# weiwei-ww/ML-VAE

Hardware: AMD Instinct MI355X
Metric: spectrogram frames/sec + ELBO; 80-d log-mel B=256 at 1/2/4/8 MI355X (higher is better)
Workload: dtype bf16

## Files before the change

ml-vae_amd/csrc/heads.hip:

```cpp
#include "common.h"
#include <stdlib.h>

namespace {

constexpr float LOG_2PI_H = 1.8378770351409912f;
constexpr int RT = 64;

struct HeadArgs {
  int B, T, N, H2, loss_type, train;
  const unsigned short* Y;
  const unsigned short* W1;
  const unsigned short* W1t;
  const float* b1;
  const float* W2[2]; const float* b2[2]; const float* W3[2]; const float* b3[2];
  const float* x; const float* lens; const int* count; float rec_scale;
  float* P1; float* P2[2]; float* OUT[2]; float* dOUT[2]; float* dP2[2]; float* dP1; float* dY;
  float* partials;
  int sbf;
  float* bias_ws;
  float* wg_ws;
};

template <int C, int F> constexpr int nbs() { return 2 * F + 2 * C + 2 * C; }

// ... 360 lines not shown
      for (int idx = tid; idx < 2 * (FK - F) * LC; idx += 256)
        sm[O_W3I + (idx / ((FK - F) * LC)) * W3R * LC + F * LC + idx % ((FK - F) * LC)] = 0;
    } else {
      for (int idx = tid; idx < 2 * C * (FK - F); idx += 256) {
        const int h = idx / (C * (FK - F)), rem = idx % (C * (FK - F));
        sm[O_W3T + h * C * LF + (rem / (FK - F)) * LF + F + rem % (FK - F)] = 0;
      }
    }
    for (int idx = tid; idx < 2 * RT * (FK - F); idx += 256) {
      const int h = idx / (RT * (FK - F)), rem = idx % (RT * (FK - F));
      sm[O_DO + h * RT * LF + (rem / (FK - F)) * LF + F + rem % (FK - F)] = 0;
    }
  }
  {
    __shared__ int cnt_sh;
    const int c = block_frames(a.lens, a.B, a.T, a.count, &cnt_sh);
    if (tid == 0) inv_cnt = c > 0 ? 1.f / ((float)c * (float)F) : 0.f;
  }

  const unsigned short* P1b = reinterpret_cast<const unsigned short*>(a.P1);
  u32x4 pn[4];
  f32x4 xn[NF];
  float lnn;
  auto prefetch = [&](int tile) {
    const int grow = tile * RT + 16 * wave + l15;
    const bool rv = tile < ntiles && grow < a.N;
    lnn = rv ? a.lens[grow / a.T] : 0.f;
#pragma unroll
    for (int i = 0; i < 4; ++i)
      pn[i] = rv ? *reinterpret_cast<const u32x4*>(P1b + (size_t)grow * C2 + 8 * (q + 4 * i)) : u32x4{0u, 0u, 0u, 0u};
#pragma unroll
    for (int j = 0; j < NF; ++j)
      xn[j] = rv ? *reinterpret_cast<const f32x4*>(a.x + (size_t)grow * F + 16 * j + 4 * q) : f32x4{0.f, 0.f, 0.f, 0.f};
  };
  prefetch(blockIdx.x);
  for (int i = tid; i < 2 * C; i += 256) sbias[i] = a.b2[i / C] ? a.b2[i / C][i % C] : 0.f;
  for (int i = tid; i < 2 * F; i += 256) sbias[2 * C + i] = a.b3[i / F] ? a.b3[i / F][i % F] : 0.f;
  __syncthreads();

  const int lrow = 16 * wave + l15;
  constexpr int NT3W = nt3<C, F>() / 4, NT2W = nt2<C, F>() / 4;
  static_assert(nt3<C, F>() % 4 == 0 && nt2<C, F>() % 4 == 0, "tiles split over 4 waves");
  f32x4 aw3[WG ? NT3W : 1], aw2[WG ? NT2W : 1];
  if constexpr (WG) {
#pragma unroll
    for (int i = 0; i < NT3W; ++i) aw3[i] = f32x4{0.f, 0.f, 0.f, 0.f};
#pragma unroll
    for (int i = 0; i < NT2W; ++i) aw2[i] = f32x4{0.f, 0.f, 0.f, 0.f};
  }
  constexpr bool SAVE = !WG;
  for (int tile = blockIdx.x; tile < ntiles; tile += gridDim.x) {
    const int grow = tile * RT + lrow;
    const bool rv = grow < a.N;
    const float lenb = lnn;
#pragma unroll
    for (int i = 0; i < 4; ++i) *reinterpret_cast<u32x4*>(sm + O_P1 + lrow * L2C + 8 * (q + 4 * i)) = pn[i];
    f32x4 xv[NF];
#pragma unroll
    for (int j = 0; j < NF; ++j) xv[j] = xn[j];
    prefetch(tile + gridDim.x);
    f32x4 p1r[NC2];
#pragma unroll
    for (int j = 0; j < NC2; ++j) {
      const bf16x4 v = *reinterpret_cast<const bf16x4*>(sm + O_P1 + lrow * L2C + 16 * j + 4 * q);
#pragma unroll
      for (int r = 0; r < 4; ++r) p1r[j][r] = bf2f(v[r]);
    }

    f32x4 acc2[2][NC], acc3[2][NF];
#pragma unroll
    for (int h = 0; h < 2; ++h) {
#pragma unroll
      for (int j = 0; j < NC; ++j) acc2[h][j] = f32x4{0.f, 0.f, 0.f, 0.f};
#pragma unroll
      for (int kk = 0; kk < C; kk += 32) {
        const bf16x8 av = lds8(sm + O_P1 + lrow * L2C + h * C + kk + 8 * q);
#pragma unroll
        for (int j = 0; j < NC; ++j) {
          acc2[h][j] = mfma16(lds8(sm + O_W2I + h * C * LC + (16 * j + l15) * LC + kk + 8 * q), av, acc2[h][j]);
          if constexpr (SPL)
            acc2[h][j] = mfma16(lds8(sm + O_W2T + h * C * LC + (16 * j + l15) * LC + kk + 8 * q), av, acc2[h][j]);
        }
      }
#pragma unroll
      for (int j = 0; j < NC; ++j) {
        const int col = 16 * j + 4 * q;
        const f32x4 bb = *reinterpret_cast<const f32x4*>(sbias + h * C + col);
#pragma unroll
        for (int r = 0; r < 4; ++r) acc2[h][j][r] = lrelu(acc2[h][j][r] + bb[r]);
        st4bf(sm + O_P2 + h * RT * LC + lrow * LC + col, acc2[h][j]);
        if (SAVE && rv) st_saved(a.P2[h], (size_t)grow * C + col, acc2[h][j], 1);
      }
#pragma unroll
      for (int j = 0; j < NF; ++j) acc3[h][j] = f32x4{0.f, 0.f, 0.f, 0.f};
#pragma unroll
      for (int kk = 0; kk < C; kk += 32) {
        const bf16x8 av = lds8(sm + O_P2 + h * RT * LC + lrow * LC + kk + 8 * q);
#pragma unroll
        for (int j = 0; j < NF; ++j) {
          const short* wr = sm + O_W3I + h * W3R * LC + (16 * j + l15) * LC;
          acc3[h][j] = mfma16(lds8(wr + kk + 8 * q), av, acc3[h][j]);
          if constexpr (SPL) {
            acc3[h][j] = mfma16(lds8(sm + O_W3T + h * F * LC + (16 * j + l15) * LC + kk + 8 * q), av, acc3[h][j]);
            const int s2 = kk / 32;
            const bf16x8 pl = {f2bf_lo(acc2[h][2 * s2][0]), f2bf_lo(acc2[h][2 * s2][1]),
                               f2bf_lo(acc2[h][2 * s2][2]), f2bf_lo(acc2[h][2 * s2][3]),
                               f2bf_lo(acc2[h][2 * s2 + 1][0]), f2bf_lo(acc2[h][2 * s2 + 1][1]),
                               f2bf_lo(acc2[h][2 * s2 + 1][2]), f2bf_lo(acc2[h][2 * s2 + 1][3])};
            const bf16x4 w0 = *reinterpret_cast<const bf16x4*>(wr + kk + 4 * q);
            const bf16x4 w1 = *reinterpret_cast<const bf16x4*>(wr + kk + 16 + 4 * q);
            acc3[h][j] = mfma16(bf16x8{w0[0], w0[1], w0[2], w0[3], w1[0], w1[1], w1[2], w1[3]}, pl, acc3[h][j]);
          }
        }
      }
#pragma unroll
      for (int j = 0; j < NF; ++j) {
        const int col = 16 * j + 4 * q;
        const f32x4 bb = *reinterpret_cast<const f32x4*>(sbias + 2 * C + h * F + col);
#pragma unroll
        for (int r = 0; r < 4; ++r) acc3[h][j][r] += bb[r];
        if (rv) *reinterpret_cast<f32x4*>(a.OUT[h] + (size_t)grow * F + col) = acc3[h][j];
      }
    }

    bool m = false;
    if (rv) m = grow % a.T < valid_frames(lenb, a.T);
    const float sc = m ? a.rec_scale * inv_cnt : 0.f;
    float lsum = 0.f;
#pragma unroll
    for (int j = 0; j < NF; ++j) {
      const int col = 16 * j + 4 * q;
      f32x4 gm, gv;
#pragma unroll
      for (int r = 0; r < 4; ++r) {
        const float mu = acc3[0][j][r], d = xv[j][r] - mu;
        float rr, gmu, glv = 0.f;
        if (lik) {
          const float lv = acc3[1][j][r];
          const float elv = expf(lv), ev = elv + 1e-5f;
          rr = 0.5f * (LOG_2PI_H + lv + d * d / ev);
          gmu = -d / ev;
          glv = 0.5f * (1.f - d * d * elv / (ev * ev));
        } else {
          rr = d * d;
          gmu = -2.f * d;
        }
        if (m) lsum += rr;
        gm[r] = sc * gmu;
        gv[r] = sc * glv;
      }
      rows16_to_lds(gm, &bred[wave][16 * j], lane);
      rows16_to_lds(gv, &bred[wave][F + 16 * j], lane);
      st4bf(sm + O_DO + lrow * LF + col, gm);
      st4bf(sm + O_DO + RT * LF + lrow * LF + col, gv);
      if (SAVE && rv) {
        st_saved(a.dOUT[0], (size_t)grow * F + col, gm, 1);
        if (lik) st_saved(a.dOUT[1], (size_t)grow * F + col, gv, 1);
      }
    }
    lsum = wave_sum(lsum);
    if (lane == 0) red[wave] = lsum;
    if constexpr (WG) {
      lds_barrier();
#pragma unroll
      for (int i = 0; i < NT3W; ++i) {
        const int t = wave * NT3W + i, h = t / ((F / 16) * NC), fb = (t / NC) % (F / 16), cb = t % NC;
        if (h < nh) {
#pragma unroll
          for (int kk = 0; kk < RT; kk += 32)
            aw3[i] = mfma16(trfrag(sm + O_DO + h * RT * LF, LF, 16 * fb, kk, lane),
                          trfrag(sm + O_P2 + h * RT * LC, LC, 16 * cb, kk, lane), aw3[i]);
        }
      }
      lds_barrier();
    }

    for (int h = 0; h < 2; ++h) {
      f32x4 acc5[NC];
#pragma unroll
      for (int j = 0; j < NC; ++j) acc5[j] = f32x4{0.f, 0.f, 0.f, 0.f};
      if (h < nh) {
#pragma unroll
        for (int kk = 0; kk < FK; kk += 32) {
          const bf16x8 av = lds8(sm + O_DO + h * RT * LF + lrow * LF + kk + 8 * q);
#pragma unroll
          for (int j = 0; j < NC; ++j)
            acc5[j] = mfma16(SPL ? trfrag(sm + O_W3I + h * W3R * LC, LC, 16 * j, kk, lane)
                               : lds8(sm + O_W3T + h * C * LF + (16 * j + l15) * LF + kk + 8 * q), av, acc5[j]);
        }
      }
#pragma unroll
      for (int j = 0; j < NC; ++j) {
        const int col = 16 * j + 4 * q;
#pragma unroll
        for (int r = 0; r < 4; ++r) acc5[j][r] *= lrelu_d(acc2[h][j][r]);
        rows16_to_lds(acc5[j], &bred[wave][2 * F + h * C + 16 * j], lane);
        st4bf(sm + O_P2 + h * RT * LC + lrow * LC + col, acc5[j]);
        if (SAVE && rv && h < nh) st_saved(a.dP2[h], (size_t)grow * C + col, acc5[j], 1);
      }
      f32x4 acc6[NC];
#pragma unroll
      for (int j = 0; j < NC; ++j) acc6[j] = f32x4{0.f, 0.f, 0.f, 0.f};
      if (h < nh) {
#pragma unroll
        for (int kk = 0; kk < C; kk += 32) {
          const bf16x8 av = lds8(sm + O_P2 + h * RT * LC + lrow * LC + kk + 8 * q);
#pragma unroll
          for (int j = 0; j < NC; ++j)
            acc6[j] = mfma16(SPL ? trfrag(sm + O_W2I + h * C * LC, LC, 16 * j, kk, lane)
                               : lds8(sm + O_W2T + h * C * LC + (16 * j + l15) * LC + kk + 8 * q), av, acc6[j]);
        }
      }
#pragma unroll
      for (int j = 0; j < NC; ++j) {
        const int col = h * C + 16 * j + 4 * q;
#pragma unroll
        for (int r = 0; r < 4; ++r) acc6[j][r] *= lrelu_d(p1r[h * NC + j][r]);
        rows16_to_lds(acc6[j], &bred[wave][2 * F + 2 * C + h * C + 16 * j], lane);
        if (rv) st_saved(a.dP1, (size_t)grow * C2 + col, acc6[j], 1);
      }
    }
    lds_barrier();
    for (int c = tid; c < NBS; c += 256)
      a.bias_ws[(size_t)tile * NBS + c] = (bred[0][c] + bred[1][c]) + (bred[2][c] + bred[3][c]);
    if (tid == 0) a.partials[tile] = red[0] + red[1] + red[2] + red[3];
    if constexpr (WG) {
#pragma unroll
      for (int i = 0; i < NT2W; ++i) {
        const int t = wave * NT2W + i, h = t / (NC * NC), ob = (t / NC) % NC, ib = t % NC;
        if (h < nh) {
#pragma unroll
          for (int kk = 0; kk < RT; kk += 32)
            aw2[i] = mfma16(trfrag(sm + O_P2 + h * RT * LC, LC, 16 * ob, kk, lane),
                          trfrag(sm + O_P1, L2C, h * C + 16 * ib, kk, lane), aw2[i]);
        }
      }
    }
    lds_barrier();
  }
  if constexpr (WG) {
    float* slab = a.wg_ws + (size_t)blockIdx.x * wg_slab<C, F>();
#pragma unroll
    for (int i = 0; i < NT3W; ++i)
      *reinterpret_cast<f32x4*>(slab + ((size_t)(wave * NT3W + i) * 64 + lane) * 4) = aw3[i];
#pragma unroll
    for (int i = 0; i < NT2W; ++i)
      *reinterpret_cast<f32x4*>(slab + ((size_t)(nt3<C, F>() + wave * NT2W + i) * 64 + lane) * 4) = aw2[i];
  }
}

constexpr int RSL = 32;
__global__ __launch_bounds__(256) void heads_bias_reduce1(int nwg, int nbs, const float* __restrict__ ws,
                                                          float* __restrict__ slices) {
  __shared__ float part[8][32];
  const int c = blockIdx.x * 32 + (threadIdx.x & 31), g = threadIdx.x >> 5, z = blockIdx.y;
  const int per = (nwg + RSL - 1) / RSL, w0 = z * per, w1 = min(nwg, w0 + per);
  float v = 0.f;
  if (c < nbs)
#pragma unroll 8
    for (int w = w0 + g; w < w1; w += 8) v += ws[(size_t)w * nbs + c];
  part[g][threadIdx.x & 31] = v;
  __syncthreads();
  if (g != 0 || c >= nbs) return;
  const int e = threadIdx.x & 31;
  slices[(size_t)z * nbs + c] = ((part[0][e] + part[1][e]) + (part[2][e] + part[3][e])) +
                                ((part[4][e] + part[5][e]) + (part[6][e] + part[7][e]));
}
__global__ __launch_bounds__(256) void heads_bias_reduce2(int nbs, int F, int C, int n1,
                                                          const float* __restrict__ slices, float* db3m,
                                                          float* db3v, float* db2m, float* db2v, float* db1) {
  const int c = blockIdx.x * 256 + threadIdx.x;
  if (c >= nbs) return;
  float t = 0.f;
#pragma unroll 8
  for (int z = 0; z < RSL; ++z) t += slices[(size_t)z * nbs + c];
  if (c < F) db3m[c] = t;
  else if (c < 2 * F) { if (db3v) db3v[c - F] = t; }
  else if (c < 2 * F + C) db2m[c - 2 * F] = t;
  else if (c < 2 * F + 2 * C) { if (db2v) db2v[c - 2 * F - C] = t; }
  else if (c - 2 * F - 2 * C < n1) db1[c - 2 * F - 2 * C] = t;
}

template <int C, int F>
int launch_heads(const HeadArgs& a, hipStream_t st) {
  constexpr int FK = (F + 31) / 32 * 32, LC = C + 8, LF = FK + 8, L2C = 2 * C + 8;
  constexpr size_t lds = (size_t)(2 * C * LC * 2 + 2 * F * LC + 2 * C * LF + RT * L2C + 2 * RT * LC +
                                  2 * RT * LF) * sizeof(short);
  auto k = heads_kernel<C, F>;
  static bool attr = false;
  if (!attr) {
    if (hipFuncSetAttribute((const void*)k, hipFuncAttributeMaxDynamicSharedMemorySize, (int)lds) !=
        hipSuccess) {
      mlvae_set_error("heads: cannot reserve %zu B LDS", lds);
      return 2;
    }
    attr = true;
  }
  k<<<(a.N + RT - 1) / RT, 256, lds, st>>>(a);
  MLVAE_CHECK_LAUNCH();
  return 0;
}

constexpr int HNT_BN = 128;
template <bool LRELU, int HNT_BK, bool SPB = false>
__global__ __launch_bounds__(512) void heads_nt_kernel(int M, int Nn, int K, const unsigned short* __restrict__ A,
                                                       int lda, const unsigned short* __restrict__ B, int ldb,
                                                       void* __restrict__ Cv, int ldc, const float* __restrict__ bias,
                                                       int out_bf16) {
  constexpr int HNT_LB = HNT_BK + 8;
  constexpr int BPT = HNT_BN * HNT_BK / 8 / 512;
  extern __shared__ __attribute__((aligned(16))) short hsm[];
  const int tid = threadIdx.x, lane = tid & 63, wave = tid >> 6, l15 = lane & 15, q = lane >> 4;
  const int nch = Nn / HNT_BN, kch = K / HNT_BK, npc = nch * kch;
  const int nblk = (M + 127) / 128;
  u32x4 bq[BPT];
  auto bload = [&](int p) {
    const int nc = p / kch, kc = p - nc * kch;
#pragma unroll
    for (int i = 0; i < BPT; ++i) {
      const int idx = tid + 512 * i, n = idx / (HNT_BK / 8), k16 = idx % (HNT_BK / 8);
      bq[i] = *reinterpret_cast<const u32x4*>(B + (size_t)(nc * HNT_BN + n) * ldb + kc * HNT_BK + 8 * k16);
    }
  };
  auto bstore = [&](int buf) {
#pragma unroll
    for (int i = 0; i < BPT; ++i) {
      const int idx = tid + 512 * i, n = idx / (HNT_BK / 8), k16 = idx % (HNT_BK / 8);
      *reinterpret_cast<u32x4*>(hsm + buf * HNT_BN * HNT_LB + n * HNT_LB + 8 * k16) = bq[i];
    }
  };
  constexpr int AKC = SPB ? HNT_BK / 2 : HNT_BK;
  auto aload = [&](bf16x8 (&af)[AKC / 32], int b, int p) {
    const int row = b * 128 + 16 * wave + l15;
    const unsigned short* arow = A + (size_t)(row < M ? row : M - 1) * lda + (p % kch) * AKC;
#pragma unroll
    for (int ks = 0; ks < AKC / 32; ++ks) af[ks] = *reinterpret_cast<const bf16x8*>(arow + 32 * ks + 8 * q);
  };
  int blk = blockIdx.x;
  if (blk >= nblk) return;
  bf16x8 afr[AKC / 32], anx[AKC / 32];
  bload(0);
  aload(afr, blk, 0);
  int buf = 0;
  f32x4 acc[HNT_BN / 16];
  for (; blk < nblk; blk += gridDim.x) {
    const int row = blk * 128 + 16 * wave + l15;
    const bool rv = row < M;
    for (int p = 0; p < npc; ++p) {
      const int nc = p / kch, kc = p - nc * kch;
      bstore(buf);
      __syncthreads();
      const int nb = p + 1 < npc ? blk : blk + (int)gridDim.x, np = p + 1 < npc ? p + 1 : 0;
      const bool more = nb < nblk, new_a = more && (kch > 1 || np == 0);
      if (more) bload(np);
      if (new_a) aload(anx, nb, np);
      if (kc == 0) {
#pragma unroll
        for (int nt = 0; nt < HNT_BN / 16; ++nt) acc[nt] = f32x4{0.f, 0.f, 0.f, 0.f};
      }
      const short* bb = hsm + buf * HNT_BN * HNT_LB;
#pragma unroll
      for (int ks = 0; ks < HNT_BK / 32; ++ks)
#pragma unroll
        for (int nt = 0; nt < HNT_BN / 16; ++nt) {
          const int brow = 32 * (nt >> 1) + 8 * (l15 >> 2) + 4 * (nt & 1) + (l15 & 3);
          acc[nt] = mfma16(*reinterpret_cast<const bf16x8*>(bb + brow * HNT_LB + 32 * ks + 8 * q),
                         afr[ks % (AKC / 32)], acc[nt]);
        }
      buf ^= 1;
      if (kc == kch - 1 && rv) {
#pragma unroll
        for (int t = 0; t < HNT_BN / 32; ++t) {
          const int col = nc * HNT_BN + 32 * t + 8 * q;
          f32x4 v0 = acc[2 * t], v1 = acc[2 * t + 1];
          if (LRELU) {
#pragma unroll
            for (int r = 0; r < 4; ++r) {
              v0[r] = lrelu(v0[r] + bias[col + r]);
              v1[r] = lrelu(v1[r] + bias[col + 4 + r]);
            }
          }
          if (out_bf16) {
            *reinterpret_cast<bf16x8*>(static_cast<unsigned short*>(Cv) + (size_t)row * ldc + col) =
                bf16x8{f2bf(v0[0]), f2bf(v0[1]), f2bf(v0[2]), f2bf(v0[3]), f2bf(v1[0]), f2bf(v1[1]), f2bf(v1[2]),
                       f2bf(v1[3])};
          } else {
            float* cr = static_cast<float*>(Cv) + (size_t)row * ldc + col;
            *reinterpret_cast<f32x4*>(cr) = v0;
            *reinterpret_cast<f32x4*>(cr + 4) = v1;
          }
        }
      }
      if (new_a) {
#pragma unroll
        for (int ks = 0; ks < AKC / 32; ++ks) afr[ks] = anx[ks];
      }
    }
  }
}

int heads_cus();
int heads_nt(bool lrelu_bias, int M, int Nn, int K, const void* A, int lda, const void* B, int ldb, void* C,
             int ldc, const float* bias, bool out_bf16, hipStream_t st, bool split_b = false) {
  if (M <= 0) return 0;
  if (Nn % HNT_BN || K % 128 || lda % 8 || ldb % 8 || ldc % 8 || (lrelu_bias && !bias) ||
      (split_b && (!lrelu_bias || ldb < 2 * K))) {
    mlvae_set_error("heads_nt: Nn %% 128, K %% 128, 16-byte rows and a bias with the LReLU epilogue");
    return 1;
  }
  constexpr size_t lds = (size_t)2 * HNT_BN * (128 + 8) * sizeof(short);
  const int nblk = (M + 127) / 128, grid = nblk < 2 * heads_cus() ? nblk : 2 * heads_cus();
  const int ki = split_b ? 2 : lrelu_bias ? 1 : 0;
  auto k = split_b ? heads_nt_kernel<true, 128, true>
                   : lrelu_bias ? heads_nt_kernel<true, 128> : heads_nt_kernel<false, 128>;
  if (split_b) K *= 2;
  static bool attr[3] = {false, false, false};
  if (!attr[ki]) {
    if (hipFuncSetAttribute((const void*)k, hipFuncAttributeMaxDynamicSharedMemorySize, (int)lds) != hipSuccess) {
      mlvae_set_error("heads_nt: cannot reserve %zu B LDS", lds);
      return 2;
    }
    attr[ki] = true;
  }
  k<<<grid, 512, lds, st>>>(M, Nn, K, static_cast<const unsigned short*>(A), lda,
                            static_cast<const unsigned short*>(B), ldb, C, ldc, bias, out_bf16 ? 1 : 0);
  MLVAE_CHECK_LAUNCH();
  return 0;
}
int g_heads_nt = [] {
  const char* e = getenv("MLVAE_HEADS_NT");
  return e ? atoi(e) : 1;
}();

int heads_cus() {
  static int n = 0;
  if (!n) {
    int dev = 0;
    if (hipGetDevice(&dev) != hipSuccess ||
        hipDeviceGetAttribute(&n, hipDeviceAttributeMultiprocessorCount, dev) != hipSuccess || n <= 0)
      n = 256;
  }
  return n;
}
int mid_grid(int N) {
  const int ntiles = (N + RT - 1) / RT, cus = heads_cus();
  return ntiles < cus ? ntiles : cus;
}

template <int C, int F, bool WG, bool SPL>
int launch_mid(const HeadArgs& a, hipStream_t st) {
  constexpr int FK = (F + 31) / 32 * 32, LC = C + 8, LF = FK + 8, L2C = 2 * C + 8;
  constexpr size_t lds = (size_t)(2 * C * LC * 2 + 2 * (SPL ? FK : F) * LC + 2 * C * LF + RT * L2C +
                                  2 * RT * LC + 2 * RT * LF) * sizeof(short);
  auto k = heads_mid_kernel<C, F, WG, SPL>;
  static bool attr = false;
  if (!attr) {
    if (hipFuncSetAttribute((const void*)k, hipFuncAttributeMaxDynamicSharedMemorySize, (int)lds) !=
        hipSuccess) {
      mlvae_set_error("heads_mid: cannot reserve %zu B LDS", lds);
      return 2;
    }
    attr = true;
  }
  k<<<mid_grid(a.N), 256, lds, st>>>(a);
  MLVAE_CHECK_LAUNCH();
  return 0;
}

constexpr int WG_NZ = 16;
__global__ __launch_bounds__(256) void heads_wg_reduce1(const float* __restrict__ slabs, int G, int S,
                                                        float* __restrict__ part) {
  const int e = blockIdx.x * 256 + threadIdx.x;
  if (e >= S) return;
  const int z = blockIdx.y, g0 = z * G / WG_NZ, g1 = (z + 1) * G / WG_NZ;
  float v = 0.f;
#pragma unroll 8
  for (int g = g0; g < g1; ++g) v += slabs[(size_t)g * S + e];
  part[(size_t)z * S + e] = v;
}
template <int C, int F>
__global__ __launch_bounds__(256) void heads_wg_reduce2(const float* __restrict__ part, float* dw3m,
                                                        float* dw3v, float* dw2m, float* dw2v) {
  constexpr int S = wg_slab<C, F>(), NC = C / 16, NF = F / 16;
  const int e = blockIdx.x * 256 + threadIdx.x;
  if (e >= S) return;
  float v = 0.f;
#pragma unroll
  for (int z = 0; z < WG_NZ; ++z) v += part[(size_t)z * S + e];
  const int r = e & 3, lane = (e >> 2) & 63, tp = e >> 8;
  const int m = 4 * (lane >> 4) + r, n = lane & 15;
  if (tp < nt3<C, F>()) {
    const int h = tp / (NF * NC), fb = (tp / NC) % NF, cb = tp % NC;
    float* d = h ? dw3v : dw3m;
    if (d) d[(16 * fb + m) * C + 16 * cb + n] = v;
  } else {
    const int t = tp - nt3<C, F>(), h = t / (NC * NC), ob = (t / NC) % NC, ib = t % NC;
    float* d = h ? dw2v : dw2m;
    if (d) d[(16 * ob + m) * C + 16 * ib + n] = v;
  }
}
template <int C, int F>
int launch_wg_reduce(const HeadArgs& a, float* dw3m, float* dw3v, float* dw2m, float* dw2v, hipStream_t st) {
  constexpr int S = wg_slab<C, F>();
  const int G = mid_grid(a.N);
  float* part = a.wg_ws + (size_t)G * S;
  heads_wg_reduce1<<<dim3((S + 255) / 256, WG_NZ), 256, 0, st>>>(a.wg_ws, G, S, part);
  MLVAE_CHECK_LAUNCH();
  heads_wg_reduce2<C, F><<<(S + 255) / 256, 256, 0, st>>>(part, dw3m, dw3v, dw2m, dw2v);
  MLVAE_CHECK_LAUNCH();
  return 0;
}

template <int C, int F>
int launch_bias_reduce(const HeadArgs& a, int n1, float* db3m, float* db3v, float* db2m, float* db2v,
                       float* db1, hipStream_t st) {
  constexpr int NBS = nbs<C, F>();
  const int nwg = (a.N + RT - 1) / RT;
  float* slices = a.bias_ws + (size_t)nwg * NBS;
  heads_bias_reduce1<<<dim3((NBS + 31) / 32, RSL), 256, 0, st>>>(nwg, NBS, a.bias_ws, slices);
  MLVAE_CHECK_LAUNCH();
  heads_bias_reduce2<<<(NBS + 255) / 256, 256, 0, st>>>(NBS, F, C, n1, slices, db3m, db3v, db2m, db2v, db1);
  MLVAE_CHECK_LAUNCH();
  return 0;
}

}

extern "C" int mlvae_gemm_bf16(int trans_a, int trans_b, int M, int N, int K, int batch,
                               const void* A, int lda, long long a_bstride, const void* B, int ldb,
                               long long b_bstride, float* C, int ldc, long long c_bstride,
                               float beta, const float* bias1, const float* bias2, int epi,
                               const float* aux, int ldaux, int kshift_T, int kshift,
                               int kshift_bstep, unsigned long long drop_seed,
                               unsigned long long drop_offset, float drop_p,
                               float* ws, size_t ws_bytes, void* stream);

extern "C" int mlvae_heads_partials_count(int B, int T) { return (B * T + RT - 1) / RT; }

extern "C" int mlvae_heads_supported(int C, int F, int H2) {
  return C == 64 && (F == 64 || F == 80) && H2 > 0 && H2 % 128 == 0;
}

extern "C" size_t mlvae_heads_bias_workspace_size(int B, int T, int F, int C) {
  return (size_t)((B * T + RT - 1) / RT + RSL) * (2 * F + 4 * C) * sizeof(float);
}

extern "C" int mlvae_heads_set_nt_mode(int mode) {
  if (mode < 0 || mode > 2) {
    mlvae_set_error("heads: nt mode %d (0 off, 1 auto, 2 always)", mode);
    return 1;
  }
  g_heads_nt = mode;
  return 0;
}
extern "C" size_t mlvae_heads_wgrad_workspace_size(int B, int T, int F, int C) {
  if (C != 64 || (F != 64 && F != 80) || B <= 0 || T <= 0) return 0;
  const size_t S = F == 80 ? wg_slab<64, 80>() : wg_slab<64, 64>();
  return ((size_t)mid_grid(B * T) + WG_NZ) * S * sizeof(float);
}

static int heads_impl(int B, int T, int F, int C, int H2, int loss_type, int train,
                      const void* y_bf16, const void* w1_bf16, const void* w1t_bf16,
                      const float* b1, const float* w2m, const float* b2m,
                      const float* w3m, const float* b3m, const float* w2v,
                      const float* b2v, const float* w3v, const float* b3v,
                      const float* x, const float* lens, const int* count,
                      float rec_scale, float* p1, float* p2m, float* p2v, float* mux,
                      float* lvx, float* dmux, float* dlvx, float* dp2m, float* dp2v,
                      float* dp1, float* dy, float* partials, float* bias_ws, size_t bias_ws_bytes,
                      float* db3m, float* db3v, float* db2m, float* db2v, float* db1, int saved_bf16,
                      float* wg_ws, size_t wg_ws_bytes, float* dw3m, float* dw3v, float* dw2m,
                      float* dw2v, const void* w1_split, void* stream);

extern "C" int mlvae_heads_fused(int B, int T, int F, int C, int H2, int loss_type, int train,
                                 const void* y_bf16, const void* w1_bf16, const void* w1t_bf16,
                                 const float* b1, const float* w2m, const float* b2m,
                                 const float* w3m, const float* b3m, const float* w2v,
                                 const float* b2v, const float* w3v, const float* b3v,
                                 const float* x, const float* lens, const int* count,
                                 float rec_scale, float* p1, float* p2m, float* p2v, float* mux,
                                 float* lvx, float* dmux, float* dlvx, float* dp2m, float* dp2v,
                                 float* dp1, float* dy, float* partials, void* stream) {
  return heads_impl(B, T, F, C, H2, loss_type, train, y_bf16, w1_bf16, w1t_bf16, b1, w2m, b2m, w3m,
                    b3m, w2v, b2v, w3v, b3v, x, lens, count, rec_scale, p1, p2m, p2v, mux, lvx, dmux,
                    dlvx, dp2m, dp2v, dp1, dy, partials, nullptr, 0, nullptr, nullptr, nullptr, nullptr,
                    nullptr, 0, nullptr, 0, nullptr, nullptr, nullptr, nullptr, nullptr, stream);
}

extern "C" int mlvae_heads_fused_ex(int B, int T, int F, int C, int H2, int loss_type, int train,
                                    const void* y_bf16, const void* w1_bf16, const void* w1t_bf16,
                                    const float* b1, const float* w2m, const float* b2m,
                                    const float* w3m, const float* b3m, const float* w2v,
                                    const float* b2v, const float* w3v, const float* b3v,
                                    const float* x, const float* lens, const int* count,
                                    float rec_scale, float* p1, float* p2m, float* p2v, float* mux,
                                    float* lvx, float* dmux, float* dlvx, float* dp2m, float* dp2v,
                                    float* dp1, float* dy, float* partials, float* bias_ws,
                                    size_t bias_ws_bytes, float* db3m, float* db3v, float* db2m,
                                    float* db2v, float* db1, int saved_bf16, void* stream) {
  return heads_impl(B, T, F, C, H2, loss_type, train, y_bf16, w1_bf16, w1t_bf16, b1, w2m, b2m, w3m,
                    b3m, w2v, b2v, w3v, b3v, x, lens, count, rec_scale, p1, p2m, p2v, mux, lvx, dmux,
                    dlvx, dp2m, dp2v, dp1, dy, partials, bias_ws, bias_ws_bytes, db3m, db3v, db2m, db2v,
                    db1, saved_bf16, nullptr, 0, nullptr, nullptr, nullptr, nullptr, nullptr, stream);
}

extern "C" int mlvae_heads_fused_ex2(int B, int T, int F, int C, int H2, int loss_type, int train,
                                     const void* y_bf16, const void* w1_bf16, const void* w1t_bf16,
                                     const float* b1, const float* w2m, const float* b2m,
                                     const float* w3m, const float* b3m, const float* w2v,
                                     const float* b2v, const float* w3v, const float* b3v,
                                     const float* x, const float* lens, const int* count,
                                     float rec_scale, float* p1, float* p2m, float* p2v, float* mux,
                                     float* lvx, float* dmux, float* dlvx, float* dp2m, float* dp2v,
                                     float* dp1, float* dy, float* partials, float* bias_ws,
                                     size_t bias_ws_bytes, float* db3m, float* db3v, float* db2m,
                                     float* db2v, float* db1, int saved_bf16, float* wg_ws,
                                     size_t wg_ws_bytes, float* dw3m, float* dw3v, float* dw2m,
                                     float* dw2v, void* stream) {
  return heads_impl(B, T, F, C, H2, loss_type, train, y_bf16, w1_bf16, w1t_bf16, b1, w2m, b2m, w3m,
                    b3m, w2v, b2v, w3v, b3v, x, lens, count, rec_scale, p1, p2m, p2v, mux, lvx, dmux,
                    dlvx, dp2m, dp2v, dp1, dy, partials, bias_ws, bias_ws_bytes, db3m, db3v, db2m, db2v,
                    db1, saved_bf16, wg_ws, wg_ws_bytes, dw3m, dw3v, dw2m, dw2v, nullptr, stream);
}

extern "C" int mlvae_heads_fused_ex3(int B, int T, int F, int C, int H2, int loss_type, int train,
                                     const void* y_bf16, const void* w1_bf16, const void* w1t_bf16,
                                     const float* b1, const float* w2m, const float* b2m,
                                     const float* w3m, const float* b3m, const float* w2v,
                                     const float* b2v, const float* w3v, const float* b3v,
                                     const float* x, const float* lens, const int* count,
                                     float rec_scale, float* p1, float* p2m, float* p2v, float* mux,
                                     float* lvx, float* dmux, float* dlvx, float* dp2m, float* dp2v,
                                     float* dp1, float* dy, float* partials, float* bias_ws,
                                     size_t bias_ws_bytes, float* db3m, float* db3v, float* db2m,
                                     float* db2v, float* db1, int saved_bf16, float* wg_ws,
                                     size_t wg_ws_bytes, float* dw3m, float* dw3v, float* dw2m,
                                     float* dw2v, const void* w1_split, void* stream) {
  return heads_impl(B, T, F, C, H2, loss_type, train, y_bf16, w1_bf16, w1t_bf16, b1, w2m, b2m, w3m,
                    b3m, w2v, b2v, w3v, b3v, x, lens, count, rec_scale, p1, p2m, p2v, mux, lvx, dmux,
                    dlvx, dp2m, dp2v, dp1, dy, partials, bias_ws, bias_ws_bytes, db3m, db3v, db2m, db2v,
                    db1, saved_bf16, wg_ws, wg_ws_bytes, dw3m, dw3v, dw2m, dw2v, w1_split, stream);
}

__global__ void bf16_split_rows_kernel(const float* __restrict__ src, int rows, int cols, int chunk,
                                       unsigned short* __restrict__ dst) {
  const long long i = (long long)blockIdx.x * 256 + threadIdx.x;
  if (i >= (long long)rows * cols) return;
  const int r = (int)(i / cols), c = (int)(i % cols), blk = c / chunk, w = c % chunk;
  const float v = src[i];
  unsigned short* d = dst + (size_t)r * 2 * cols + (size_t)blk * 2 * chunk + w;
  d[0] = (unsigned short)f2bf(v);
  d[chunk] = (unsigned short)f2bf_lo(v);
}
extern "C" int mlvae_bf16_split_rows(const float* src, int rows, int cols, int chunk, void* dst, void* stream) {
  if (rows <= 0 || cols <= 0) return 0;
  if (!src || !dst || chunk <= 0 || cols % chunk) {
    mlvae_set_error("mlvae_bf16_split_rows: null pointer or cols %% chunk");
    return 1;
  }
  const long long n = (long long)rows * cols;
  bf16_split_rows_kernel<<<(unsigned)((n + 255) / 256), 256, 0, (hipStream_t)stream>>>(
      src, rows, cols, chunk, static_cast<unsigned short*>(dst));
  MLVAE_CHECK_LAUNCH();
  return 0;
}

static int heads_impl(int B, int T, int F, int C, int H2, int loss_type, int train,
                                 const void* y_bf16, const void* w1_bf16, const void* w1t_bf16,
                                 const float* b1, const float* w2m, const float* b2m,
                                 const float* w3m, const float* b3m, const float* w2v,
                                 const float* b2v, const float* w3v, const float* b3v,
                                 const float* x, const float* lens, const int* count,
                                 float rec_scale, float* p1, float* p2m, float* p2v, float* mux,
                                 float* lvx, float* dmux, float* dlvx, float* dp2m, float* dp2v,
                                 float* dp1, float* dy, float* partials, float* bias_ws, size_t bias_ws_bytes,
                                 float* db3m, float* db3v, float* db2m, float* db2v, float* db1,
                                 int saved_bf16, float* wg_ws, size_t wg_ws_bytes, float* dw3m, float* dw3v,
                                 float* dw2m, float* dw2v, const void* w1_split, void* stream) {
  if (B <= 0 || T <= 0) return 0;
  if (!mlvae_heads_supported(C, F, H2)) {
    mlvae_set_error("heads: unsupported shape C=%d F=%d 2H=%d (C 64, F 64|80, 2H %% 128)", C, F, H2);
    return 1;
  }
  if (loss_type != 0 && loss_type != 1) { mlvae_set_error("Invalid loss type: %d", loss_type); return 1; }
  if (!y_bf16 || !w1_bf16 || !b1 || !w2m || !w3m || !w2v || !w3v || !b2m || !b3m || !b2v || !b3v ||
      !x || !lens || !mux || !lvx || !partials ||
      (train && (!w1t_bf16 || !p1 || !p2m || !p2v || !dmux || (loss_type == 0 && !dlvx) || !dp2m ||
                 !dp2v || !dp1 || !dy))) {
    mlvae_set_error("heads: null pointer");
    return 1;
  }
  HeadArgs a;
  a.B = B; a.T = T; a.N = B * T; a.H2 = H2; a.loss_type = loss_type; a.train = train;
  a.Y = static_cast<const unsigned short*>(y_bf16);
  a.W1 = static_cast<const unsigned short*>(w1_bf16);
  a.W1t = static_cast<const unsigned short*>(w1t_bf16);
  a.b1 = b1;
  a.W2[0] = w2m; a.b2[0] = b2m; a.W3[0] = w3m; a.b3[0] = b3m;
  a.W2[1] = w2v; a.b2[1] = b2v; a.W3[1] = w3v; a.b3[1] = b3v;
  a.x = x; a.lens = lens; a.count = count; a.rec_scale = rec_scale;
  a.P1 = p1; a.P2[0] = p2m; a.P2[1] = p2v; a.OUT[0] = mux; a.OUT[1] = lvx;
  a.dOUT[0] = dmux; a.dOUT[1] = dlvx; a.dP2[0] = dp2m; a.dP2[1] = dp2v; a.dP1 = dp1; a.dY = dy;
  a.partials = partials;
  a.sbf = (saved_bf16 & 1) ? 1 : 0;
  const bool dy_bf16 = (saved_bf16 & 2) != 0;
  a.bias_ws = nullptr;
  if (bias_ws) {
    const bool mse = loss_type == 1;
    if (!train || bias_ws_bytes < mlvae_heads_bias_workspace_size(B, T, F, C) || !db3m || !db2m || !db1 ||
        (!mse && (!db3v || !db2v))) {
      mlvae_set_error("heads: bias sums need train, a workspace of %zu B and the bias gradients",
                      mlvae_heads_bias_workspace_size(B, T, F, C));
      return 1;
    }
    a.bias_ws = bias_ws;
  }
  hipStream_t st = (hipStream_t)stream;
  int rc;
  const bool split = train && bias_ws && (saved_bf16 & 1);
  a.wg_ws = nullptr;
  if (wg_ws) {
    const bool mse = loss_type == 1;
    if (!split || wg_ws_bytes < mlvae_heads_wgrad_workspace_size(B, T, F, C) || !dw3m || !dw2m ||
        (!mse && (!dw3v || !dw2v))) {
      mlvae_set_error("heads: fused weight gradients need the split form, a workspace of %zu B and "
// ... 48 lines not shown
```

Measured before the change: 13.46 million.

## Rework heads NT GEMM with buffer loads, LDS bias, deferred stores and ping-pong A

Rewrites the heads NT GEMM kernel to use raw buffer loads and stores with bounds-checked resources, which removes the row clamping and validity branches. The bias is staged in LDS once per block, and bf16 output stores are deferred so they overlap the next tile's MFMA work. Two A-fragment register sets alternate in a K-major ping-pong loop, and the kernel is pinned to 4 waves per EU. In exchange it adds template variants, more LDS, and new limits on leading dimensions, with some risk of register pressure or spills.

```diff
diff --git a/ml-vae_amd/csrc/heads.hip b/ml-vae_amd/csrc/heads.hip
--- a/ml-vae_amd/csrc/heads.hip
+++ b/ml-vae_amd/csrc/heads.hip
@@ -686,8 +686,9 @@
 }
 
 constexpr int HNT_BN = 128;
-template <bool LRELU, int HNT_BK, bool SPB = false>
-__global__ __launch_bounds__(512) void heads_nt_kernel(int M, int Nn, int K, const unsigned short* __restrict__ A,
+template <bool LRELU, int HNT_BK, bool SPB = false, bool KM = true>
+__global__ __launch_bounds__(512) __attribute__((amdgpu_waves_per_eu(4, 4)))
+void heads_nt_kernel(int M, int Nn, int K, const unsigned short* __restrict__ A,
                                                        int lda, const unsigned short* __restrict__ B, int ldb,
                                                        void* __restrict__ Cv, int ldc, const float* __restrict__ bias,
                                                        int out_bf16) {
@@ -697,14 +698,22 @@
   const int tid = threadIdx.x, lane = tid & 63, wave = tid >> 6, l15 = lane & 15, q = lane >> 4;
   const int nch = Nn / HNT_BN, kch = K / HNT_BK, npc = nch * kch;
   const int nblk = (M + 127) / 128;
+  int blk = blockIdx.x;
+  if (blk >= nblk) return;
+  const float* sbias = reinterpret_cast<const float*>(hsm + 2 * HNT_BN * HNT_LB);
+  if (LRELU) {
+    for (int i = tid; i < Nn; i += 512) reinterpret_cast<float*>(hsm + 2 * HNT_BN * HNT_LB)[i] = bias[i];
+  }
   u32x4 bq[BPT];
+  const unsigned boff = (unsigned)((tid / (HNT_BK / 8)) * ldb + 8 * (tid % (HNT_BK / 8))) * 2u;
+  const unsigned bstep = (unsigned)(512 / (HNT_BK / 8) * ldb) * 2u;
   auto bload = [&](int p) {
     const int nc = p / kch, kc = p - nc * kch;
-#pragma unroll
-    for (int i = 0; i < BPT; ++i) {
-      const int idx = tid + 512 * i, n = idx / (HNT_BK / 8), k16 = idx % (HNT_BK / 8);
-      bq[i] = *reinterpret_cast<const u32x4*>(B + (size_t)(nc * HNT_BN + n) * ldb + kc * HNT_BK + 8 * k16);
-    }
+    const auto rb = make_rsrc(B + (size_t)nc * HNT_BN * ldb + kc * HNT_BK,
+                              (unsigned)((HNT_BN - 1) * ldb + HNT_BK) * 2u);
+#pragma unroll
+    for (int i = 0; i < BPT; ++i)
+      bq[i] = __builtin_bit_cast(u32x4, __builtin_amdgcn_raw_buffer_load_b128(rb, boff, i * bstep, 0));
   };
   auto bstore = [&](int buf) {
 #pragma unroll
@@ -714,73 +723,116 @@
     }
   };
   constexpr int AKC = SPB ? HNT_BK / 2 : HNT_BK;
-  auto aload = [&](bf16x8 (&af)[AKC / 32], int b, int p) {
-    const int row = b * 128 + 16 * wave + l15;
-    const unsigned short* arow = A + (size_t)(row < M ? row : M - 1) * lda + (p % kch) * AKC;
-#pragma unroll
-    for (int ks = 0; ks < AKC / 32; ++ks) af[ks] = *reinterpret_cast<const bf16x8*>(arow + 32 * ks + 8 * q);
+  constexpr int NA = AKC / 32;
+  const unsigned aoff = (unsigned)((16 * wave + l15) * lda + 8 * q) * 2u;
+  auto aload = [&](bf16x8 (&af)[NA], int b, int kc) {
+    const int rows = min(128, M - b * 128);
+    const auto ra = make_rsrc(A + (rows > 0 ? (size_t)b * 128 * lda + kc * AKC : 0),
+                              rows > 0 ? (unsigned)((rows - 1) * lda + AKC) * 2u : 0u);
+#pragma unroll
+    for (int ks = 0; ks < NA; ++ks)
+      af[ks] = __builtin_bit_cast(bf16x8, __builtin_amdgcn_raw_buffer_load_b128(ra, aoff + 64 * ks, 0, 0));
   };
-  int blk = blockIdx.x;
-  if (blk >= nblk) return;
-  bf16x8 afr[AKC / 32], anx[AKC / 32];
-  bload(0);
-  aload(afr, blk, 0);
-  int buf = 0;
+  auto c_rsrc = [&](int b, int nc, int esz) {
+    const int rows = min(128, M - b * 128);
+    return make_rsrc(static_cast<char*>(Cv) + ((size_t)b * 128 * ldc + nc * HNT_BN) * esz,
+                     (unsigned)((rows - 1) * ldc + HNT_BN) * (unsigned)esz);
+  };
+  const unsigned coff = (unsigned)((16 * wave + l15) * ldc + 8 * q);
+  int p = 0, buf = 0;
   f32x4 acc[HNT_BN / 16];
-  for (; blk < nblk; blk += gridDim.x) {
-    const int row = blk * 128 + 16 * wave + l15;
-    const bool rv = row < M;
-    for (int p = 0; p < npc; ++p) {
-      const int nc = p / kch, kc = p - nc * kch;
-      bstore(buf);
-      __syncthreads();
-      const int nb = p + 1 < npc ? blk : blk + (int)gridDim.x, np = p + 1 < npc ? p + 1 : 0;
-      const bool more = nb < nblk, new_a = more && (kch > 1 || np == 0);
-      if (more) bload(np);
-      if (new_a) aload(anx, nb, np);
-      if (kc == 0) {
-#pragma unroll
-        for (int nt = 0; nt < HNT_BN / 16; ++nt) acc[nt] = f32x4{0.f, 0.f, 0.f, 0.f};
-      }
-      const short* bb = hsm + buf * HNT_BN * HNT_LB;
-#pragma unroll
-      for (int ks = 0; ks < HNT_BK / 32; ++ks)
-#pragma unroll
-        for (int nt = 0; nt < HNT_BN / 16; ++nt) {
-          const int brow = 32 * (nt >> 1) + 8 * (l15 >> 2) + 4 * (nt & 1) + (l15 & 3);
-          acc[nt] = mfma16(*reinterpret_cast<const bf16x8*>(bb + brow * HNT_LB + 32 * ks + 8 * q),
-                         afr[ks % (AKC / 32)], acc[nt]);
-        }
-      buf ^= 1;
-      if (kc == kch - 1 && rv) {
-#pragma unroll
-        for (int t = 0; t < HNT_BN / 32; ++t) {
+  constexpr bool DEFER = !KM || !SPB;
+  u32x4 pq[HNT_BN / 32];
+  auto prs = make_rsrc(Cv, 0u);
+#pragma unroll
+  for (int t = 0; t < HNT_BN / 32; ++t) pq[t] = u32x4{0u, 0u, 0u, 0u};
+  auto flush = [&]() {
+    if constexpr (!DEFER) return;
+#pragma unroll
+    for (int t = 0; t < HNT_BN / 32; ++t) __builtin_amdgcn_raw_buffer_store_b128(pq[t], prs, 2u * coff + 64 * t, 0, 0);
+    prs = make_rsrc(Cv, 0u);
+  };
+  auto piece = [&](bf16x8 (&use)[NA], bf16x8 (&ld)[NA]) {
+    const int nc = p / kch, kc = p - nc * kch;
+    bstore(buf);
+    __syncthreads();
+    const bool last = p + 1 == npc;
+    const int nb = last ? blk + (int)gridDim.x : blk, np = last ? 0 : p + 1;
+    bload(np);
+    bool new_a = false;
+    if constexpr (KM) {
+      aload(ld, nb, np % kch);
+    } else {
+      new_a = last && nb < nblk;
+      if (new_a) aload(ld, nb, 0);
+    }
+    if (!KM || kc == 0) flush();
+    if (kc == 0) {
+#pragma unroll
+      for (int nt = 0; nt < HNT_BN / 16; ++nt) acc[nt] = f32x4{0.f, 0.f, 0.f, 0.f};
+    }
+    const short* bb = hsm + buf * HNT_BN * HNT_LB;
+#pragma unroll
+    for (int ks = 0; ks < HNT_BK / 32; ++ks)
+#pragma unroll
+      for (int nt = 0; nt < HNT_BN / 16; ++nt) {
+        const int brow = 32 * (nt >> 1) + 8 * (l15 >> 2) + 4 * (nt & 1) + (l15 & 3);
+        acc[nt] = mfma16(*reinterpret_cast<const bf16x8*>(bb + brow * HNT_LB + 32 * ks + 8 * q), use[ks % NA],
+                         acc[nt]);
+      }
+    buf ^= 1;
+    if (kc == kch - 1) {
+      const auto rc = c_rsrc(blk, nc, out_bf16 ? 2 : 4);
+#pragma unroll
+      for (int t = 0; t < HNT_BN / 32; ++t) {
+        f32x4 v0 = acc[2 * t], v1 = acc[2 * t + 1];
+        if (LRELU) {
           const int col = nc * HNT_BN + 32 * t + 8 * q;
-          f32x4 v0 = acc[2 * t], v1 = acc[2 * t + 1];
-          if (LRELU) {
-#pragma unroll
-            for (int r = 0; r < 4; ++r) {
-              v0[r] = lrelu(v0[r] + bias[col + r]);
-              v1[r] = lrelu(v1[r] + bias[col + 4 + r]);
-            }
-          }
-          if (out_bf16) {
-            *reinterpret_cast<bf16x8*>(static_cast<unsigned short*>(Cv) + (size_t)row * ldc + col) =
-                bf16x8{f2bf(v0[0]), f2bf(v0[1]), f2bf(v0[2]), f2bf(v0[3]), f2bf(v1[0]), f2bf(v1[1]), f2bf(v1[2]),
-                       f2bf(v1[3])};
-          } else {
-            float* cr = static_cast<float*>(Cv) + (size_t)row * ldc + col;
-            *reinterpret_cast<f32x4*>(cr) = v0;
-            *reinterpret_cast<f32x4*>(cr + 4) = v1;
+          const f32x4 b0 = *reinterpret_cast<const f32x4*>(sbias + col);
+          const f32x4 b1 = *reinterpret_cast<const f32x4*>(sbias + col + 4);
+#pragma unroll
+          for (int r = 0; r < 4; ++r) {
+            v0[r] = lrelu(v0[r] + b0[r]);
+            v1[r] = lrelu(v1[r] + b1[r]);
           }
         }
-      }
-      if (new_a) {
-#pragma unroll
-        for (int ks = 0; ks < AKC / 32; ++ks) afr[ks] = anx[ks];
-      }
-    }
-  }
+        if (out_bf16) {
+          const u32x4 o = __builtin_bit_cast(u32x4, bf16x8{f2bf(v0[0]), f2bf(v0[1]), f2bf(v0[2]), f2bf(v0[3]),
+                                                           f2bf(v1[0]), f2bf(v1[1]), f2bf(v1[2]), f2bf(v1[3])});
+          if constexpr (DEFER) pq[t] = o;
+          else __builtin_amdgcn_raw_buffer_store_b128(o, rc, 2u * coff + 64 * t, 0, 0);
+        } else {
+          __builtin_amdgcn_raw_buffer_store_b128(__builtin_bit_cast(u32x4, v0), rc, 4u * coff + 128 * t, 0, 0);
+          __builtin_amdgcn_raw_buffer_store_b128(__builtin_bit_cast(u32x4, v1), rc, 4u * coff + 128 * t + 16, 0, 0);
+        }
+      }
+      if (DEFER && out_bf16) prs = rc;
+    }
+    if (new_a) {
+#pragma unroll
+      for (int ks = 0; ks < NA; ++ks) use[ks] = ld[ks];
+    }
+    blk = nb;
+    p = np;
+  };
+  bf16x8 a0[NA], a1[NA];
+  bload(0);
+  __builtin_amdgcn_sched_barrier(0);
+  aload(a0, blk, 0);
+  __builtin_amdgcn_sched_barrier(0);
+  flush();
+  __builtin_amdgcn_sched_barrier(0);
+  if constexpr (KM) {
+    for (;;) {
+      piece(a0, a1);
+      if (blk >= nblk) break;
+      piece(a1, a0);
+      if (blk >= nblk) break;
+    }
+  } else {
+    while (blk < nblk) piece(a0, a1);
+  }
+  flush();
 }
 
 int heads_cus();
@@ -788,23 +840,26 @@
              int ldc, const float* bias, bool out_bf16, hipStream_t st, bool split_b = false) {
   if (M <= 0) return 0;
   if (Nn % HNT_BN || K % 128 || lda % 8 || ldb % 8 || ldc % 8 || (lrelu_bias && !bias) ||
-      (split_b && (!lrelu_bias || ldb < 2 * K))) {
+      (split_b && (!lrelu_bias || ldb < 2 * K)) || lda < K || ldb < K || ldc < Nn ||
+      lda >= (1 << 22) || ldb >= (1 << 22) || ldc >= (1 << 22)) {
     mlvae_set_error("heads_nt: Nn %% 128, K %% 128, 16-byte rows and a bias with the LReLU epilogue");
     return 1;
   }
-  constexpr size_t lds = (size_t)2 * HNT_BN * (128 + 8) * sizeof(short);
+  const size_t lds = (size_t)2 * HNT_BN * (128 + 8) * sizeof(short) + (lrelu_bias ? Nn * sizeof(float) : 0);
   const int nblk = (M + 127) / 128, grid = nblk < 2 * heads_cus() ? nblk : 2 * heads_cus();
-  const int ki = split_b ? 2 : lrelu_bias ? 1 : 0;
-  auto k = split_b ? heads_nt_kernel<true, 128, true>
-                   : lrelu_bias ? heads_nt_kernel<true, 128> : heads_nt_kernel<false, 128>;
   if (split_b) K *= 2;
-  static bool attr[3] = {false, false, false};
-  if (!attr[ki]) {
+  const bool km = K > 128;
+  const int ki = split_b ? 4 : (lrelu_bias ? 2 : 0) + (km ? 1 : 0);
+  auto k = split_b ? heads_nt_kernel<true, 128, true, true>
+           : lrelu_bias ? (km ? heads_nt_kernel<true, 128, false, true> : heads_nt_kernel<true, 128, false, false>)
+                        : (km ? heads_nt_kernel<false, 128, false, true> : heads_nt_kernel<false, 128, false, false>);
+  static size_t attr[5] = {0, 0, 0, 0, 0};
+  if (attr[ki] < lds) {
     if (hipFuncSetAttribute((const void*)k, hipFuncAttributeMaxDynamicSharedMemorySize, (int)lds) != hipSuccess) {
       mlvae_set_error("heads_nt: cannot reserve %zu B LDS", lds);
       return 2;
     }
-    attr[ki] = true;
+    attr[ki] = lds;
   }
   k<<<grid, 512, lds, st>>>(M, Nn, K, static_cast<const unsigned short*>(A), lda,
                             static_cast<const unsigned short*>(B), ldb, C, ldc, bias, out_bf16 ? 1 : 0);
```

Result: no change. 13.76 million, median of 6 (+2.2%).
